# ahoynodnarb/minidiff

Measured on AMD Instinct MI355X. Metric: forward+backward passes/sec on 4096x4096 fp32 matmul+elementwise graph, higher is better.
Workload: dtype f32

## Files before the change

minidiff_amd/csrc/gemm_bf16x3.hip:

```cpp
#include "md_hip.h"
#include "md_bf16x3.h"
#include "md_bf16x3_layout.h"

namespace {

typedef __attribute__((address_space(3))) void bx_lds_void;
typedef __attribute__((address_space(1))) const void bx_gbl_void;
typedef __bf16 bx_bf16x8 __attribute__((ext_vector_type(8)));
typedef int bx_i32x4 __attribute__((ext_vector_type(4)));
typedef float bx_f32x4 __attribute__((ext_vector_type(4)));
typedef float bx_f32x16 __attribute__((ext_vector_type(16)));

constexpr int BX_BM = 256, BX_BN = 128, BX_BK = 32;
constexpr int BX_NT = 512;
constexpr int BX_ROWB = BX_BK * 2;

__device__ __forceinline__ bool bx_split8(const float (&x)[8], bx_i32x4 *q1, bx_i32x4 *q2, bx_i32x4 *q3) {
  bool bad = false;
  uint32_t h[3][8];
#pragma unroll
  for (int j = 0; j < 8; ++j) {
    uint32_t p1, p2, p3;
    bad |= md_bf16x3_split(x[j], &p1, &p2, &p3);
    h[0][j] = p1 >> 16; h[1][j] = p2 >> 16; h[2][j] = p3 >> 16;
  }
  bx_i32x4 *q[3] = {q1, q2, q3};
#pragma unroll
  for (int p = 0; p < 3; ++p)
#pragma unroll
    for (int w = 0; w < 4; ++w) (*q[p])[w] = (int)(h[p][2 * w] | (h[p][2 * w + 1] << 16));
  return bad;
}

__global__ void __launch_bounds__(256) k_bf16x3_split_rows(const float *__restrict__ src, int64_t rows, int64_t K, int64_t rs, char *__restrict__ dst,
                                                           int64_t plane, unsigned *flag) {
  bool bad = false;
  const int64_t k = ((int64_t)blockIdx.x * 256 + threadIdx.x) * 8;
  if (k < K) {
    for (int64_t r = blockIdx.y; r < rows; r += gridDim.y) {
      const bx_f32x4 lo = *(const bx_f32x4 *)(src + r * rs + k), hi = *(const bx_f32x4 *)(src + r * rs + k + 4);
      const float x[8] = {lo[0], lo[1], lo[2], lo[3], hi[0], hi[1], hi[2], hi[3]};
      bx_i32x4 q1, q2, q3;
      bad |= bx_split8(x, &q1, &q2, &q3);
      char *d = dst + md_bf16x3_plane_off(r, k, K * 2, 64);
      *(bx_i32x4 *)d = q1; *(bx_i32x4 *)(d + plane) = q2; *(bx_i32x4 *)(d + 2 * plane) = q3;
    }
  }
  if (__syncthreads_or(bad) && threadIdx.x == 0) atomicOr(flag, 1u);
}

__global__ void __launch_bounds__(256) k_bf16x3_split_rows_kt(const float *__restrict__ src, int64_t rows, int64_t K, int64_t rs, char *__restrict__ dst,
                                                              int64_t plane, unsigned *flag) {
  bool bad = false;
  const int l = threadIdx.x & 63, w = threadIdx.x >> 6;
  const int64_t k = (((int64_t)blockIdx.x * 4 + w) * 8 + (l >> 3)) * 32 + (l & 3) * 8;
  if (k < K) {
    for (int64_t r = (int64_t)blockIdx.y * 2 + ((l >> 2) & 1); r < rows; r += (int64_t)gridDim.y * 2) {
      const bx_f32x4 lo = *(const bx_f32x4 *)(src + r * rs + k), hi = *(const bx_f32x4 *)(src + r * rs + k + 4);
      const float x[8] = {lo[0], lo[1], lo[2], lo[3], hi[0], hi[1], hi[2], hi[3]};
      bx_i32x4 q1, q2, q3;
      bad |= bx_split8(x, &q1, &q2, &q3);
      char *d = dst + md_bf16x3_plane_off(r, k, 64, rows * 64);
      *(bx_i32x4 *)d = q1; *(bx_i32x4 *)(d + plane) = q2; *(bx_i32x4 *)(d + 2 * plane) = q3;
    }
  }
  if (__syncthreads_or(bad) && threadIdx.x == 0) atomicOr(flag, 1u);
}

__global__ void __launch_bounds__(256) k_bf16x3_split_cols(const float *__restrict__ src, int64_t rows, int64_t K, int64_t ks, char *__restrict__ dst,
                                                           int64_t plane, int64_t prs, int64_t pks, unsigned *flag) {
  __shared__ float T[32][66];
  const int t = threadIdx.x;
  for (int64_t kb = blockIdx.y; kb < K / 32; kb += gridDim.y) {
    const int64_t r0 = (int64_t)blockIdx.x * 64, k0 = kb * 32;
#pragma unroll
    for (int i = 0; i < 2; ++i) {
      const int idx = t + 256 * i, kk = idx >> 4, r4 = (idx & 15) * 4;
      const bx_f32x4 v = *(const bx_f32x4 *)(src + (k0 + kk) * ks + r0 + r4);
      T[kk][r4] = v[0]; T[kk][r4 + 1] = v[1]; T[kk][r4 + 2] = v[2]; T[kk][r4 + 3] = v[3];
    }
    __syncthreads();
    const int kg = t & 3, r = t >> 2;
    float x[8];
#pragma unroll
    for (int j = 0; j < 8; ++j) x[j] = T[kg * 8 + j][r];
    bx_i32x4 q1, q2, q3;
    const bool bad = bx_split8(x, &q1, &q2, &q3);
    char *d = dst + md_bf16x3_plane_off(r0 + r, k0 + kg * 8, prs, pks);
    *(bx_i32x4 *)d = q1; *(bx_i32x4 *)(d + plane) = q2; *(bx_i32x4 *)(d + 2 * plane) = q3;
    if (__syncthreads_or(bad) && t == 0) atomicOr(flag, 1u);
  }
}

template <int NP>
__device__ __forceinline__ bool bxp_split8(const float (&x)[8], bx_i32x4 (&q)[NP]) {
  bool bad = false;
  uint32_t h[NP][8];
#pragma unroll
  for (int j = 0; j < 8; ++j) {
    uint32_t p[2];
    bad |= md_bf16x3_split_rn(x[j], NP, &p[0], &p[1]);
#pragma unroll
    for (int i = 0; i < NP; ++i) h[i][j] = p[i] >> 16;
  }
#pragma unroll
  for (int p = 0; p < NP; ++p)
#pragma unroll
    for (int w = 0; w < 4; ++w) q[p][w] = (int)(h[p][2 * w] | (h[p][2 * w + 1] << 16));
  return bad;
}
template <int NP>
__device__ __forceinline__ void bxp_put(char *d, int64_t plane, const bx_i32x4 (&q)[NP]) {
#pragma unroll
  for (int p = 0; p < NP; ++p) *(bx_i32x4 *)(d + p * plane) = q[p];
}

template <int NP>
__global__ void __launch_bounds__(256) k_bf16xp_split_rows(const float *__restrict__ src, int64_t rows, int64_t K, int64_t rs, char *__restrict__ dst,
                                                           int64_t plane, unsigned *flag) {
  bool bad = false;
  const int64_t k = ((int64_t)blockIdx.x * 256 + threadIdx.x) * 8;
  if (k < K) {
    for (int64_t r = blockIdx.y; r < rows; r += gridDim.y) {
      const bx_f32x4 lo = *(const bx_f32x4 *)(src + r * rs + k), hi = *(const bx_f32x4 *)(src + r * rs + k + 4);
      const float x[8] = {lo[0], lo[1], lo[2], lo[3], hi[0], hi[1], hi[2], hi[3]};
      bx_i32x4 q[NP];
      bad |= bxp_split8<NP>(x, q);
      bxp_put<NP>(dst + md_bf16x3_plane_off(r, k, K * 2, 64), plane, q);
    }
  }
  if (__syncthreads_or(bad) && threadIdx.x == 0) atomicOr(flag, 1u);
}

template <int NP>
__global__ void __launch_bounds__(256) k_bf16xp_split_rows_kt(const float *__restrict__ src, int64_t rows, int64_t K, int64_t rs, char *__restrict__ dst,
                                                              int64_t plane, unsigned *flag) {
  bool bad = false;
  const int l = threadIdx.x & 63, w = threadIdx.x >> 6;
  const int64_t k = (((int64_t)blockIdx.x * 4 + w) * 8 + (l >> 3)) * 32 + (l & 3) * 8;
  if (k < K) {
    for (int64_t r = (int64_t)blockIdx.y * 2 + ((l >> 2) & 1); r < rows; r += (int64_t)gridDim.y * 2) {
      const bx_f32x4 lo = *(const bx_f32x4 *)(src + r * rs + k), hi = *(const bx_f32x4 *)(src + r * rs + k + 4);
      const float x[8] = {lo[0], lo[1], lo[2], lo[3], hi[0], hi[1], hi[2], hi[3]};
      bx_i32x4 q[NP];
      bad |= bxp_split8<NP>(x, q);
      bxp_put<NP>(dst + md_bf16x3_plane_off(r, k, 64, rows * 64), plane, q);
    }
  }
  if (__syncthreads_or(bad) && threadIdx.x == 0) atomicOr(flag, 1u);
}

template <int NP>
__global__ void __launch_bounds__(256) k_bf16xp_split_cols(const float *__restrict__ src, int64_t rows, int64_t K, int64_t ks, char *__restrict__ dst,
                                                           int64_t plane, int64_t prs, int64_t pks, unsigned *flag) {
  __shared__ float T[32][66];
  const int t = threadIdx.x;
  for (int64_t kb = blockIdx.y; kb < K / 32; kb += gridDim.y) {
    const int64_t r0 = (int64_t)blockIdx.x * 64, k0 = kb * 32;
#pragma unroll
    for (int i = 0; i < 2; ++i) {
      const int idx = t + 256 * i, kk = idx >> 4, r4 = (idx & 15) * 4;
      const bx_f32x4 v = *(const bx_f32x4 *)(src + (k0 + kk) * ks + r0 + r4);
      T[kk][r4] = v[0]; T[kk][r4 + 1] = v[1]; T[kk][r4 + 2] = v[2]; T[kk][r4 + 3] = v[3];
    }
    __syncthreads();
    const int kg = t & 3, r = t >> 2;
    float x[8];
#pragma unroll
    for (int j = 0; j < 8; ++j) x[j] = T[kg * 8 + j][r];
    bx_i32x4 q[NP];
    const bool bad = bxp_split8<NP>(x, q);
    bxp_put<NP>(dst + md_bf16x3_plane_off(r0 + r, k0 + kg * 8, prs, pks), plane, q);
    if (__syncthreads_or(bad) && t == 0) atomicOr(flag, 1u);
  }
}

struct Bx3Args {
  const char *A, *B;
  float *C;
  int64_t K, c_ms;
  int64_t a_plane, b_plane;
  int64_t rs, a_kstep, b_kstep;
  int tiles_m, tiles_n, gm;
  const unsigned *flag;
  unsigned long long *stamp;
};

__device__ __forceinline__ const char *bx_uniform(const char *p) {
  uint32_t lo = (uint32_t)(uintptr_t)p, hi = (uint32_t)((uintptr_t)p >> 32);
  asm("" : "+s"(lo), "+s"(hi));
  return reinterpret_cast<const char *>(((uintptr_t)hi << 32) | lo);
}

__device__ __forceinline__ void bx_piece(const char *P, int64_t rs, int64_t row, int64_t kstep, int kt, uint32_t lane_off, char *S) {
  uint32_t off = lane_off;
  asm("" : "+v"(off) : "s"(kt));
  const char *src = bx_uniform(P + row * rs + kt * kstep) + off;
  __builtin_amdgcn_global_load_lds((bx_gbl_void *)src, (bx_lds_void *)S, 16, 0, 0);
}

struct Bx3Bufs { char *a[3], *b[3]; };

template <int NP>
__device__ __forceinline__ void bx_stage(const Bx3Args &g, int64_t m0, int64_t n0, int kt, const Bx3Bufs &S, uint32_t lane_off) {
  const int wave = __builtin_amdgcn_readfirstlane(threadIdx.x >> 6);
#pragma unroll
  for (int p = 0; p < NP; ++p) {
#pragma unroll
    for (int i = 0; i < 2; ++i) bx_piece(g.A + p * g.a_plane, g.rs, m0 + 16 * (wave + 8 * i), g.a_kstep, kt, lane_off, S.a[p] + (wave + 8 * i) * 1024);
    bx_piece(g.B + p * g.b_plane, g.rs, n0 + 16 * wave, g.b_kstep, kt, lane_off, S.b[p] + wave * 1024);
  }
}

__device__ __forceinline__ bx_bf16x8 bx_frag(const char *S, int rb, int s) {
  const int l = threadIdx.x & 63, r = rb + (l & 31), c = 2 * s + (l >> 5);
  return __builtin_bit_cast(bx_bf16x8, *(const bx_i32x4 *)(S + r * BX_ROWB + ((c ^ ((r >> 2) & 3)) << 4)));
}

__device__ __forceinline__ bx_bf16x8 bx_frag_at(const char *S, uint32_t off, int half) {
  return __builtin_bit_cast(bx_bf16x8, *(const bx_i32x4 *)(S + off + half * 32 * BX_ROWB));
}
__device__ __forceinline__ uint32_t bx_read_off(int rb, int s) {
  const int l = threadIdx.x & 63, r = rb + (l & 31), c = 2 * s + (l >> 5);
  return (uint32_t)(r * BX_ROWB + ((c ^ ((r >> 2) & 3)) << 4));
}

template <int NP, int NPROD>
__device__ __forceinline__ void bx_mma(const Bx3Bufs &S, int wm, int wn, bx_f32x16 (&acc)[2][2]) {
  bx_f32x16 part[2][2];
#pragma unroll
  for (int i = 0; i < 2; ++i)
#pragma unroll
    for (int j = 0; j < 2; ++j)
#pragma unroll
      for (int e = 0; e < 16; ++e) part[i][j][e] = 0;
#pragma unroll
  for (int s = 0; s < 2; ++s) {
    bx_bf16x8 a[NP][2], b[NP][2];
#pragma unroll
    for (int p = 0; p < NP; ++p)
#pragma unroll
      for (int i = 0; i < 2; ++i) {
        a[p][i] = bx_frag(S.a[p], wm * 64 + i * 32, s);
        b[p][i] = bx_frag(S.b[p], wn * 64 + i * 32, s);
      }
    constexpr int PA[6] = {0, 0, 1, 0, 1, 2}, PB[6] = {0, 1, 0, 2, 1, 0};
#pragma unroll
    for (int q = 0; q < NPROD; ++q)
#pragma unroll
      for (int i = 0; i < 2; ++i)
#pragma unroll
        for (int j = 0; j < 2; ++j) part[i][j] = __builtin_amdgcn_mfma_f32_32x32x16_bf16(a[PA[q]][i], b[PB[q]][j], part[i][j], 0, 0, 0);
  }
#pragma unroll
  for (int i = 0; i < 2; ++i)
#pragma unroll
    for (int j = 0; j < 2; ++j) acc[i][j] += part[i][j];
}

struct Bx3Src { const char *a[3][2], *b[3]; };
struct Bx3Dst { char *a[3][2], *b[3]; };

__device__ __forceinline__ void bx_fence() { __builtin_amdgcn_sched_barrier(0); }

__device__ __forceinline__ void bx_dma(const char *&base, int64_t step, uint32_t lane_off, char *S) {
  base = bx_uniform(base + step);
  uint32_t off = lane_off;
  asm("" : "+v"(off));
  __builtin_amdgcn_global_load_lds((bx_gbl_void *)(base + off), (bx_lds_void *)S, 16, 0, 0);
}

__device__ __forceinline__ void bx_dma_n(Bx3Src &src, const Bx3Dst &dst, int n, int64_t ka, int64_t kb, uint32_t lane_off) {
  const int p = n / 3, i = n % 3;
  if (i < 2) bx_dma(src.a[p][i], ka, lane_off, dst.a[p][i]);
  else bx_dma(src.b[p], kb, lane_off, dst.b[p]);
}

__device__ __forceinline__ void bx_fold4(bx_f32x16 &acc, const bx_f32x16 &part, int e0) {
  float r0 = acc[e0] + part[e0], r1 = acc[e0 + 1] + part[e0 + 1], r2 = acc[e0 + 2] + part[e0 + 2], r3 = acc[e0 + 3] + part[e0 + 3];
  asm volatile("" : "+v"(r0), "+v"(r1), "+v"(r2), "+v"(r3));
  acc[e0] = r0; acc[e0 + 1] = r1; acc[e0 + 2] = r2; acc[e0 + 3] = r3;
}

template <bool STAGE>
__device__ __forceinline__ void bx_tile(const Bx3Bufs &S, Bx3Src &src, const Bx3Dst &dst, int64_t ka, int64_t kb, uint32_t lane_off, const uint32_t (&rd)[4],
                                        bx_f32x16 (&acc)[2][2], bx_f32x16 &carry) {
  constexpr int PA[6] = {0, 0, 1, 0, 1, 2}, PB[6] = {0, 1, 0, 2, 1, 0};
  bx_f32x16 part[2][2];
  bx_bf16x8 a0[3][2], b0[3][2], a1[3][2], b1[3][2];
  uint32_t ra0 = rd[0], ra1 = rd[1], rb0 = rd[2], rb1 = rd[3];
  asm volatile("" : "+v"(ra0), "+v"(ra1), "+v"(rb0), "+v"(rb1));
  a0[0][0] = bx_frag_at(S.a[0], ra0, 0); b0[0][0] = bx_frag_at(S.b[0], rb0, 0); b0[0][1] = bx_frag_at(S.b[0], rb0, 1); a0[0][1] = bx_frag_at(S.a[0], ra0, 1);
  b0[1][0] = bx_frag_at(S.b[1], rb0, 0); b0[1][1] = bx_frag_at(S.b[1], rb0, 1);
  a0[1][0] = bx_frag_at(S.a[1], ra0, 0); a0[1][1] = bx_frag_at(S.a[1], ra0, 1);
  b0[2][0] = bx_frag_at(S.b[2], rb0, 0); b0[2][1] = bx_frag_at(S.b[2], rb0, 1);
  a0[2][0] = bx_frag_at(S.a[2], ra0, 0); a0[2][1] = bx_frag_at(S.a[2], ra0, 1);
  bx_fence();
#pragma unroll
  for (int q = 0; q < 6; ++q)
#pragma unroll
    for (int i = 0; i < 2; ++i)
#pragma unroll
      for (int j = 0; j < 2; ++j) {
        const int n = q * 4 + i * 2 + j;
        if (q == 0) {
          const bx_f32x16 zero = {0, 0, 0, 0, 0, 0, 0, 0, 0, 0, 0, 0, 0, 0, 0, 0};
          part[i][j] = __builtin_amdgcn_mfma_f32_32x32x16_bf16(a0[0][i], b0[0][j], zero, 0, 0, 0);
        } else {
          part[i][j] = __builtin_amdgcn_mfma_f32_32x32x16_bf16(a0[PA[q]][i], b0[PB[q]][j], part[i][j], 0, 0, 0);
        }
        if (n < 4) bx_fold4(acc[1][1], carry, 4 * n);
        if (n >= 4 && n <= 12) {
          if (STAGE) bx_dma_n(src, dst, n - 4, ka, kb, lane_off);
          if (n == 12) __builtin_amdgcn_s_waitcnt(0xC07F);
        }
        switch (n) {
          case 12: a1[0][0] = bx_frag_at(S.a[0], ra1, 0); b1[0][0] = bx_frag_at(S.b[0], rb1, 0); break;
          case 13: b1[1][0] = bx_frag_at(S.b[1], rb1, 0); a1[1][0] = bx_frag_at(S.a[1], ra1, 0); break;
          case 14: b1[2][0] = bx_frag_at(S.b[2], rb1, 0); a1[2][0] = bx_frag_at(S.a[2], ra1, 0); break;
          case 15: b1[0][1] = bx_frag_at(S.b[0], rb1, 1); b1[1][1] = bx_frag_at(S.b[1], rb1, 1); break;
          case 16: b1[2][1] = bx_frag_at(S.b[2], rb1, 1); a1[0][1] = bx_frag_at(S.a[0], ra1, 1); break;
          case 17: a1[1][1] = bx_frag_at(S.a[1], ra1, 1); a1[2][1] = bx_frag_at(S.a[2], ra1, 1); break;
          default: break;
        }
        bx_fence();
      }
#pragma unroll
  for (int t = 0; t < 4; ++t) {
    const int i = t >> 1, j = t & 1;
#pragma unroll
    for (int q = 0; q < 6; ++q) {
      part[i][j] = __builtin_amdgcn_mfma_f32_32x32x16_bf16(a1[PA[q]][i], b1[PB[q]][j], part[i][j], 0, 0, 0);
      if (t > 0 && q >= 2) bx_fold4(acc[(t - 1) >> 1][(t - 1) & 1], part[(t - 1) >> 1][(t - 1) & 1], 4 * (q - 2));
      bx_fence();
    }
  }
  carry = part[1][1];
}

__device__ __forceinline__ void bx2_barrier() {
  bx_fence();
  asm volatile("" ::: "memory");
  __builtin_amdgcn_s_barrier();
  asm volatile("" ::: "memory");
  bx_fence();
}

template <bool STAGE>
__device__ __forceinline__ void bx2_tile(const Bx3Bufs &S, Bx3Src &src, const Bx3Dst &dst, int64_t ka, int64_t kb, uint32_t lane_off, const uint32_t (&rd)[4],
                                         bx_f32x16 (&acc)[2][2], bx_f32x16 (&part)[2][2]) {
  constexpr int PA[6] = {0, 0, 1, 0, 1, 2}, PB[6] = {0, 1, 0, 2, 1, 0};
  constexpr int NL = 3, CSTEP = 4;
#pragma unroll
  for (int s = 0; s < 2; ++s) {
    bx_bf16x8 a[3][2], b[3][2];
    uint32_t ra = rd[s], rb = rd[2 + s];
    asm volatile("" : "+v"(ra), "+v"(rb));
    a[0][0] = bx_frag_at(S.a[0], ra, 0); b[0][0] = bx_frag_at(S.b[0], rb, 0); b[0][1] = bx_frag_at(S.b[0], rb, 1); a[0][1] = bx_frag_at(S.a[0], ra, 1);
    b[1][0] = bx_frag_at(S.b[1], rb, 0); b[1][1] = bx_frag_at(S.b[1], rb, 1);
    a[1][0] = bx_frag_at(S.a[1], ra, 0); a[1][1] = bx_frag_at(S.a[1], ra, 1);
    b[2][0] = bx_frag_at(S.b[2], rb, 0); b[2][1] = bx_frag_at(S.b[2], rb, 1);
    a[2][0] = bx_frag_at(S.a[2], ra, 0); a[2][1] = bx_frag_at(S.a[2], ra, 1);
    bx_fence();
    if (s == 0) {
      if (STAGE) {
#pragma unroll
        for (int n = 0; n < NL; ++n) bx_dma_n(src, dst, n, ka, kb, lane_off);
      }
      bx_fence();
#pragma unroll
      for (int t = 0; t < 4; ++t)
#pragma unroll
        for (int e = 0; e < 16; e += 4) bx_fold4(acc[t >> 1][t & 1], part[t >> 1][t & 1], e);
      bx_fence();
    }
    if (s == 0) __builtin_amdgcn_s_waitcnt(0xC07F);
    else __builtin_amdgcn_s_waitcnt(0x0070);
    bx2_barrier();
#pragma unroll
    for (int q = 0; q < 6; ++q)
#pragma unroll
      for (int i = 0; i < 2; ++i)
#pragma unroll
        for (int j = 0; j < 2; ++j) {
          const int n = q * 4 + i * 2 + j;
          if (s == 0 && q == 0) {
            const bx_f32x16 zero = {0, 0, 0, 0, 0, 0, 0, 0, 0, 0, 0, 0, 0, 0, 0, 0};
            part[i][j] = __builtin_amdgcn_mfma_f32_32x32x16_bf16(a[0][i], b[0][j], zero, 0, 0, 0);
          } else {
            part[i][j] = __builtin_amdgcn_mfma_f32_32x32x16_bf16(a[PA[q]][i], b[PB[q]][j], part[i][j], 0, 0, 0);
          }
          if (STAGE && s == 0 && n % CSTEP == 1 && NL + n / CSTEP < 9) bx_dma_n(src, dst, NL + n / CSTEP, ka, kb, lane_off);
          bx_fence();
        }
    bx2_barrier();
  }
}

__device__ __forceinline__ void bx_origin(const Bx3Args &g, int64_t *m0, int64_t *n0) {
  const int nwg = g.tiles_m * g.tiles_n, bid = blockIdx.x, xcd = bid & 7, q = nwg >> 3, r = nwg & 7;
  const int wg = (xcd < r ? xcd * (q + 1) : r * (q + 1) + (xcd - r) * q) + (bid >> 3);
  int tm, tn;
  md_bf16x3_tile(wg, g.tiles_m, g.tiles_n, g.gm, &tm, &tn);
  *m0 = (int64_t)tm * BX_BM; *n0 = (int64_t)tn * BX_BN;
}
__device__ __forceinline__ void bx_write_c(const Bx3Args &g, int64_t m0, int64_t n0, int wm, int wn, int l, const bx_f32x16 (&acc)[2][2]) {
#pragma unroll
  for (int i = 0; i < 2; ++i)
#pragma unroll
    for (int j = 0; j < 2; ++j)
#pragma unroll
      for (int e = 0; e < 16; ++e) {
        const int64_t m = m0 + wm * 64 + i * 32 + (e & 3) + 8 * (e >> 2) + 4 * (l >> 5), n = n0 + wn * 64 + j * 32 + (l & 31);
        g.C[m * g.c_ms + n] = acc[i][j][e];
      }
}

template <int LOOP, bool STAMP = false>
__global__ void __launch_bounds__(BX_NT) k_gemm_bf16x3(Bx3Args g) {
  __shared__ __attribute__((aligned(16))) char sA00[BX_BM * BX_ROWB];
  __shared__ __attribute__((aligned(16))) char sA01[BX_BM * BX_ROWB];
  __shared__ __attribute__((aligned(16))) char sA02[BX_BM * BX_ROWB];
  __shared__ __attribute__((aligned(16))) char sB00[BX_BN * BX_ROWB];
  __shared__ __attribute__((aligned(16))) char sB01[BX_BN * BX_ROWB];
  __shared__ __attribute__((aligned(16))) char sB02[BX_BN * BX_ROWB];
  __shared__ __attribute__((aligned(16))) char sA10[BX_BM * BX_ROWB];
  __shared__ __attribute__((aligned(16))) char sA11[BX_BM * BX_ROWB];
  __shared__ __attribute__((aligned(16))) char sA12[BX_BM * BX_ROWB];
  __shared__ __attribute__((aligned(16))) char sB10[BX_BN * BX_ROWB];
  __shared__ __attribute__((aligned(16))) char sB11[BX_BN * BX_ROWB];
  __shared__ __attribute__((aligned(16))) char sB12[BX_BN * BX_ROWB];
  if (g.flag && *g.flag != 0) return;
  const Bx3Bufs S0{{sA00, sA01, sA02}, {sB00, sB01, sB02}}, S1{{sA10, sA11, sA12}, {sB10, sB11, sB12}};
  const int nwg = g.tiles_m * g.tiles_n, bid = blockIdx.x, xcd = bid & 7, q = nwg >> 3, r = nwg & 7;
  const int wg = (xcd < r ? xcd * (q + 1) : r * (q + 1) + (xcd - r) * q) + (bid >> 3);
  int tm, tn;
  md_bf16x3_tile(wg, g.tiles_m, g.tiles_n, g.gm, &tm, &tn);
  const int64_t m0 = (int64_t)tm * BX_BM, n0 = (int64_t)tn * BX_BN;
  const int wave = threadIdx.x >> 6, wm = wave >> 1, wn = wave & 1, l = threadIdx.x & 63;
  const int nk = (int)(g.K / BX_BK);
  const uint32_t lane_off = (uint32_t)((l >> 2) * g.rs + (((l & 3) ^ ((l >> 4) & 3)) << 4));
  bx_f32x16 acc[2][2];
#pragma unroll
  for (int i = 0; i < 2; ++i)
#pragma unroll
    for (int j = 0; j < 2; ++j)
#pragma unroll
      for (int e = 0; e < 16; ++e) acc[i][j][e] = 0;
  unsigned long long st_c = 0, st_r = 0;
  if constexpr (STAMP) {
    st_c = __builtin_amdgcn_s_memtime(); st_r = __builtin_amdgcn_s_memrealtime();
    __builtin_amdgcn_s_waitcnt(0xC07F);
  }
  if constexpr (LOOP == 0) {
    bx_stage<3>(g, m0, n0, 0, S0, lane_off);
    for (int kt = 0; kt < nk; kt += 2) {
      __syncthreads();
      if (kt + 1 < nk) bx_stage<3>(g, m0, n0, kt + 1, S1, lane_off);
      bx_mma<3, 6>(S0, wm, wn, acc);
      if (kt + 1 >= nk) break;
      __syncthreads();
      if (kt + 2 < nk) bx_stage<3>(g, m0, n0, kt + 2, S0, lane_off);
      bx_mma<3, 6>(S1, wm, wn, acc);
    }
  } else {
    const int uw = __builtin_amdgcn_readfirstlane(wave);
    const int64_t rs = g.rs, ka = g.a_kstep, kb = g.b_kstep;
    Bx3Src src;
    Bx3Dst d0, d1;
#pragma unroll
    for (int p = 0; p < 3; ++p) {
#pragma unroll
      for (int i = 0; i < 2; ++i) {
        src.a[p][i] = bx_uniform(g.A + p * g.a_plane + (m0 + 16 * (uw + 8 * i)) * rs);
        d0.a[p][i] = S0.a[p] + (uw + 8 * i) * 1024;
        d1.a[p][i] = S1.a[p] + (uw + 8 * i) * 1024;
      }
      src.b[p] = bx_uniform(g.B + p * g.b_plane + (n0 + 16 * uw) * rs);
      d0.b[p] = S0.b[p] + uw * 1024;
      d1.b[p] = S1.b[p] + uw * 1024;
    }
    const uint32_t rd[4] = {bx_read_off(wm * 64, 0), bx_read_off(wm * 64, 1), bx_read_off(wn * 64, 0), bx_read_off(wn * 64, 1)};
    if constexpr (LOOP == 1) {
      bx_f32x16 carry = {0, 0, 0, 0, 0, 0, 0, 0, 0, 0, 0, 0, 0, 0, 0, 0};
#pragma unroll
      for (int n = 0; n < 9; ++n) bx_dma_n(src, d0, n, 0, 0, lane_off);
      int kt = 0;
      for (; kt + 2 < nk; kt += 2) {
        __syncthreads();
        bx_tile<true>(S0, src, d1, ka, kb, lane_off, rd, acc, carry);
        __syncthreads();
        bx_tile<true>(S1, src, d0, ka, kb, lane_off, rd, acc, carry);
      }
      __syncthreads();
      if (kt + 1 < nk) {
        bx_tile<true>(S0, src, d1, ka, kb, lane_off, rd, acc, carry);
        __syncthreads();
        bx_tile<false>(S1, src, d0, 0, 0, lane_off, rd, acc, carry);
      } else {
        bx_tile<false>(S0, src, d1, 0, 0, lane_off, rd, acc, carry);
      }
#pragma unroll
      for (int e = 0; e < 16; e += 4) bx_fold4(acc[1][1], carry, e);
    } else {
      const int half = uw >> 2;
      bx_f32x16 part[2][2];
#pragma unroll
      for (int i = 0; i < 2; ++i)
#pragma unroll
        for (int j = 0; j < 2; ++j)
#pragma unroll
          for (int e = 0; e < 16; ++e) part[i][j][e] = 0;
#pragma unroll
      for (int n = 0; n < 9; ++n) bx_dma_n(src, d0, n, 0, 0, lane_off);
      __builtin_amdgcn_s_waitcnt(0x0070);
      bx2_barrier();
      if (half) bx2_barrier();
      int kt = 0;
      for (; kt + 2 < nk; kt += 2) {
        bx2_tile<true>(S0, src, d1, ka, kb, lane_off, rd, acc, part);
        bx2_tile<true>(S1, src, d0, ka, kb, lane_off, rd, acc, part);
      }
      if (kt + 1 < nk) {
        bx2_tile<true>(S0, src, d1, ka, kb, lane_off, rd, acc, part);
        bx2_tile<false>(S1, src, d0, 0, 0, lane_off, rd, acc, part);
      } else {
        bx2_tile<false>(S0, src, d1, 0, 0, lane_off, rd, acc, part);
      }
#pragma unroll
      for (int t = 0; t < 4; ++t)
#pragma unroll
        for (int e = 0; e < 16; e += 4) bx_fold4(acc[t >> 1][t & 1], part[t >> 1][t & 1], e);
      if (!half) bx2_barrier();
    }
  }
  if constexpr (STAMP) {
    if (threadIdx.x == 0) {
      g.stamp[2 * blockIdx.x] = __builtin_amdgcn_s_memtime() - st_c;
      g.stamp[2 * blockIdx.x + 1] = __builtin_amdgcn_s_memrealtime() - st_r;
    }
  }
#pragma unroll
  for (int i = 0; i < 2; ++i)
#pragma unroll
    for (int j = 0; j < 2; ++j)
#pragma unroll
      for (int e = 0; e < 16; ++e) {
        const int64_t m = m0 + wm * 64 + i * 32 + (e & 3) + 8 * (e >> 2) + 4 * (l >> 5), n = n0 + wn * 64 + j * 32 + (l & 31);
        g.C[m * g.c_ms + n] = acc[i][j][e];
      }
}

template <int NPROD>
__global__ void __launch_bounds__(BX_NT) k_gemm_bf16xp(Bx3Args g) {
  constexpr int NP = NPROD == 1 ? 1 : 2;
  __shared__ __attribute__((aligned(16))) char sA0[NP * BX_BM * BX_ROWB];
  __shared__ __attribute__((aligned(16))) char sB0[NP * BX_BN * BX_ROWB];
  __shared__ __attribute__((aligned(16))) char sA1[NP * BX_BM * BX_ROWB];
  __shared__ __attribute__((aligned(16))) char sB1[NP * BX_BN * BX_ROWB];
  if (g.flag && *g.flag != 0) return;
  const Bx3Bufs S0{{sA0, sA0 + (NP - 1) * BX_BM * BX_ROWB, nullptr}, {sB0, sB0 + (NP - 1) * BX_BN * BX_ROWB, nullptr}};
  const Bx3Bufs S1{{sA1, sA1 + (NP - 1) * BX_BM * BX_ROWB, nullptr}, {sB1, sB1 + (NP - 1) * BX_BN * BX_ROWB, nullptr}};
  int64_t m0, n0;
  bx_origin(g, &m0, &n0);
  const int wave = threadIdx.x >> 6, wm = wave >> 1, wn = wave & 1, l = threadIdx.x & 63;
  const int nk = (int)(g.K / BX_BK);
  const uint32_t lane_off = (uint32_t)((l >> 2) * g.rs + (((l & 3) ^ ((l >> 4) & 3)) << 4));
  bx_f32x16 acc[2][2];
#pragma unroll
  for (int i = 0; i < 2; ++i)
#pragma unroll
    for (int j = 0; j < 2; ++j)
#pragma unroll
      for (int e = 0; e < 16; ++e) acc[i][j][e] = 0;
  bx_stage<NP>(g, m0, n0, 0, S0, lane_off);
  for (int kt = 0; kt < nk; kt += 2) {
    __syncthreads();
    if (kt + 1 < nk) bx_stage<NP>(g, m0, n0, kt + 1, S1, lane_off);
    bx_mma<NP, NPROD>(S0, wm, wn, acc);
    if (kt + 1 >= nk) break;
    __syncthreads();
    if (kt + 2 < nk) bx_stage<NP>(g, m0, n0, kt + 2, S0, lane_off);
    bx_mma<NP, NPROD>(S1, wm, wn, acc);
  }
  bx_write_c(g, m0, n0, wm, wn, l, acc);
}

}

int md_gemm_bf16x3_split(const float *src, bool k_contig, int64_t rows, int64_t K, int64_t stride, void *planes, unsigned *flag, int layout, int nplanes) {
  const int64_t plane = rows * K * 2;
  char *dst = (char *)planes;
  if (k_contig && layout) {
    const dim3 grid((unsigned)((K / 32 + 31) / 32), (unsigned)(rows / 2 < 65535 ? rows / 2 : 65535));
    switch (nplanes) {
      case 1: k_bf16xp_split_rows_kt<1><<<grid, 256, 0, md_stream()>>>(src, rows, K, stride, dst, plane, flag); break;
      case 2: k_bf16xp_split_rows_kt<2><<<grid, 256, 0, md_stream()>>>(src, rows, K, stride, dst, plane, flag); break;
      default: k_bf16x3_split_rows_kt<<<grid, 256, 0, md_stream()>>>(src, rows, K, stride, dst, plane, flag); break;
    }
  } else if (k_contig) {
    const dim3 grid((unsigned)((K / 8 + 255) / 256), (unsigned)(rows < 65535 ? rows : 65535));
    switch (nplanes) {
      case 1: k_bf16xp_split_rows<1><<<grid, 256, 0, md_stream()>>>(src, rows, K, stride, dst, plane, flag); break;
      case 2: k_bf16xp_split_rows<2><<<grid, 256, 0, md_stream()>>>(src, rows, K, stride, dst, plane, flag); break;
      default: k_bf16x3_split_rows<<<grid, 256, 0, md_stream()>>>(src, rows, K, stride, dst, plane, flag); break;
    }
  } else {
    const dim3 grid((unsigned)(rows / 64), (unsigned)(K / 32 < 65535 ? K / 32 : 65535));
    const int64_t prs = md_bf16x3_row_stride(layout, K), pks = md_bf16x3_k_step(layout, rows);
    switch (nplanes) {
      case 1: k_bf16xp_split_cols<1><<<grid, 256, 0, md_stream()>>>(src, rows, K, stride, dst, plane, prs, pks, flag); break;
      case 2: k_bf16xp_split_cols<2><<<grid, 256, 0, md_stream()>>>(src, rows, K, stride, dst, plane, prs, pks, flag); break;
      default: k_bf16x3_split_cols<<<grid, 256, 0, md_stream()>>>(src, rows, K, stride, dst, plane, prs, pks, flag); break;
    }
  }
  return MD_LAUNCH_CHECK("matmul(bf16x3 split)");
}

int md_gemm_bf16x3(const void *a_planes, const void *b_planes, float *c, int64_t M, int64_t N, int64_t K, int64_t c_ms, const unsigned *flag, int loop,
                   int layout, int band, int products, unsigned long long *stamp) {
  Bx3Args a{};
  a.A = (const char *)a_planes; a.B = (const char *)b_planes; a.C = c;
  a.K = K; a.c_ms = c_ms;
  a.a_plane = M * K * 2; a.b_plane = N * K * 2;
  a.rs = md_bf16x3_row_stride(layout, K); a.a_kstep = md_bf16x3_k_step(layout, M); a.b_kstep = md_bf16x3_k_step(layout, N);
  a.tiles_m = (int)(M / BX_BM); a.tiles_n = (int)(N / BX_BN);
  a.gm = md_bf16x3_band(a.tiles_m, MD_NUM_CUS / 8, band);
  a.flag = flag;
  a.stamp = stamp;
  md_opt_table()[MD_OPT_GEMM_BF16X3_RUNS] += 1;
  const dim3 grid((unsigned)(a.tiles_m * a.tiles_n));
  if (products == 1) MD_LAUNCH(k_gemm_bf16xp<1>, grid, BX_NT, a);
  else if (products == 3) MD_LAUNCH(k_gemm_bf16xp<3>, grid, BX_NT, a);
  else if (stamp && loop == 0) MD_LAUNCH((k_gemm_bf16x3<0, true>), grid, BX_NT, a);
  else if (stamp && loop == 2) MD_LAUNCH((k_gemm_bf16x3<2, true>), grid, BX_NT, a);
  else if (stamp) MD_LAUNCH((k_gemm_bf16x3<1, true>), grid, BX_NT, a);
  else if (loop == 0) MD_LAUNCH(k_gemm_bf16x3<0>, grid, BX_NT, a);
  else if (loop == 2) MD_LAUNCH(k_gemm_bf16x3<2>, grid, BX_NT, a);
  else MD_LAUNCH(k_gemm_bf16x3<1>, grid, BX_NT, a);
  return MD_LAUNCH_CHECK("matmul(f32 as bf16x3)");
}
```

minidiff_amd/csrc/md_options.h:

```cpp
#pragma once
#include <stdint.h>
#include <stdlib.h>
#include <string.h>

#define MD_OPTION_LIST(X)                                                                                                        \
                                                                                    \
  X(PINNED_CAP, "pinned_cap", (int64_t)4 << 30, 'c')                  \
  X(JIT, "jit", 1, 'c')                                      \
  X(JIT_VERBOSE, "jit_verbose", 0, 'c')                                           \
  X(INDEX_DEFER, "index_defer", 0, 'c')                 \
                                                              \
  X(JIT_MIN, "jit_min", 1 << 18, 'x')                                   \
  X(COMM_PRIORITY, "comm_priority", 0, 'x')                         \
  X(MAX_BLOCKS, "max_blocks", 0, 'x')                                      \
  X(NT, "nt", -1, 'x')                                      \
  X(GEMM_CFG, "gemm_cfg", -1, 'x')                                  \
  X(GEMM_GLDS, "gemm_glds", 1, 'x')                                                   \
  X(GEMM_NBUF, "gemm_nbuf", 0, 'x')                     \
  X(GEMM_PEEL, "gemm_peel", 1, 'x')                            \
  X(GEMM_TT_SWAP, "gemm_tt_swap", 1, 'x')                                \
  X(GEMM_REPACK, "gemm_repack", 1, 'x')                         \
  X(GEMM_SUPER, "gemm_super", 8, 'x')                                      \
  X(GEMM_SPLITK, "gemm_splitk", 1, 'x')                                                                                         \
  X(GEMM_STAMP, "gemm_stamp", 0, 'x')                                                  \
  X(GEMM_F64_MFMA, "gemm_f64_mfma", 1, 'x')                                                                                     \
  X(GEMM_SKINNY, "gemm_skinny", 1, 'x')                                \
  X(GEMM_WIDEN, "gemm_widen", 1, 'x')                   \
  X(GEMM_NARROW_SKINNY, "gemm_narrow_skinny", 1, 'x')   \
  X(GEMM_NARROW_THIN_RUNS, "gemm_narrow_thin_runs", 0, 'x')  \
  X(GEMM_BF16X3, "gemm_bf16x3", 1, 'x')                 \
  X(GEMM_BF16X3_RUNS, "gemm_bf16x3_runs", 0, 'x')       \
  X(GEMM_BF16X3_LOOP, "gemm_bf16x3_loop", 2, 'x')       \
  X(GEMM_BF16X3_BAND, "gemm_bf16x3_band", 0, 'x')       \
  X(GEMM_BF16X3_PLANES, "gemm_bf16x3_planes", 1, 'x')   \
  X(GEMM_PRODUCTS, "gemm_products", 6, 'x')             \
  X(JIT_U, "jit_u", 0, 'x')                             \
  X(JIT_BLOCKS, "jit_blocks", 0, 'x')                                       \
  X(JIT_AXES_WIDE, "jit_axes_wide", 0, 'x')             \
  X(SWEEP_NB, "sweep_nb", 0, 'x')                                         \
  X(SWEEP_RU, "sweep_ru", 0, 'x')                                                                                               \
  X(SWEEP_NT_STORE, "sweep_nt_store", 1, 'x')                                                                                   \
  X(ROWS_WAVE, "rows_wave", 1, 'x')                                                                                             \
  X(COLS_NB, "cols_nb", 0, 'x')                                                                                                 \
  X(ROWS_BLOCKS, "rows_blocks", 0, 'x')                                          \
  X(ARG_BLOCKS, "arg_blocks", 0, 'x')                                   \
  X(ARG_BATCHED, "arg_batched", 1, 'x')                 \
  X(VAR_BATCHED, "var_batched", 1, 'x')                      \
  X(GATHER_RUNS, "gather_runs", 1, 'x')                                                                                         \
  X(SCATTER_CENSUS, "scatter_census", 1, 'x')                                                                                   \
  X(SCATTER_SORTED, "scatter_sorted", 1, 'x')

enum MdOptId {
#define MD_OPT_ENUM(ID, name, dflt, kind) MD_OPT_##ID,
  MD_OPTION_LIST(MD_OPT_ENUM)
#undef MD_OPT_ENUM
  MD_OPT_COUNT
};

struct MdOptDef {
  const char *name;
  int64_t dflt;
  char kind;
};

inline const MdOptDef *md_opt_defs() {
  static const MdOptDef defs[MD_OPT_COUNT] = {
#define MD_OPT_DEF(ID, name, dflt, kind) {name, (int64_t)(dflt), kind},
      MD_OPTION_LIST(MD_OPT_DEF)
#undef MD_OPT_DEF
  };
  return defs;
}

inline int64_t *md_opt_table() {
  static int64_t table[MD_OPT_COUNT];
  static const bool loaded = [] {
    const MdOptDef *d = md_opt_defs();
    const char *ex = getenv("MDHIP_EXPERIMENTS");
    const bool experiments = ex && ex[0] == '1' && ex[1] == 0;
    for (int i = 0; i < MD_OPT_COUNT; ++i) {
      table[i] = d[i].dflt;
      if (d[i].kind == 'x' && !experiments) continue;
      char env[64] = "MDHIP_";
      size_t n = strlen(env);
      for (const char *p = d[i].name; *p && n + 1 < sizeof env; ++p) env[n++] = (char)((*p >= 'a' && *p <= 'z') ? *p - 32 : *p);
      env[n] = 0;
      if (const char *v = getenv(env)) table[i] = (int64_t)atoll(v);
    }
    return true;
  }();
  (void)loaded;
  return table;
}
inline int64_t md_opt(int id) { return md_opt_table()[id]; }
inline int md_opt_find(const char *name) {
  const MdOptDef *d = md_opt_defs();
  for (int i = 0; i < MD_OPT_COUNT; ++i)
    if (strcmp(d[i].name, name) == 0) return i;
  return -1;
}
```

Before: 608.7.

## Add 16x16x32 MFMA bf16x3 loop variant with split accumulators and make default

```diff
diff --git a/minidiff_amd/csrc/gemm_bf16x3.hip b/minidiff_amd/csrc/gemm_bf16x3.hip
--- a/minidiff_amd/csrc/gemm_bf16x3.hip
+++ b/minidiff_amd/csrc/gemm_bf16x3.hip
@@ -397,6 +397,86 @@
   }
 }
 
+__device__ __forceinline__ uint32_t bx3_swz(int g) { return (0x78u >> (2 * g)) & 3u; }
+
+__device__ __forceinline__ uint32_t bx3_read_off(int rb) {
+  const int l = threadIdx.x & 63, r = rb + (l & 15), c = l >> 4;
+  return (uint32_t)(r * BX_ROWB + ((c ^ bx3_swz((r >> 2) & 3)) << 4));
+}
+__device__ __forceinline__ bx_bf16x8 bx3_frag_at(const char *S, uint32_t off, int i) {
+  return __builtin_bit_cast(bx_bf16x8, *(const bx_i32x4 *)(S + off + i * 16 * BX_ROWB));
+}
+
+__device__ __forceinline__ void bx3_fold4(bx_f32x4 &acc, const bx_f32x4 &part) {
+  float r0 = acc[0] + part[0], r1 = acc[1] + part[1], r2 = acc[2] + part[2], r3 = acc[3] + part[3];
+  asm volatile("" : "+v"(r0), "+v"(r1), "+v"(r2), "+v"(r3));
+  acc[0] = r0; acc[1] = r1; acc[2] = r2; acc[3] = r3;
+}
+
+template <bool STAGE>
+__device__ __forceinline__ void bx3_tile(const Bx3Bufs &S, Bx3Src &src, const Bx3Dst &dst, int64_t ka, int64_t kb, uint32_t lane_off, const uint32_t (&rd)[2],
+                                         bx_f32x4 (&acc)[4][4], bx_f32x4 (&part)[2][4]) {
+  constexpr int PA[6] = {0, 0, 1, 0, 1, 2}, PB[6] = {0, 1, 0, 2, 1, 0};
+  constexpr int NL = 3, CSTEP = 8;
+  bx_bf16x8 b[3][4];
+#pragma unroll
+  for (int h = 0; h < 2; ++h) {
+    bx_bf16x8 a[3][2];
+    uint32_t ra = rd[0], rb = rd[1];
+    asm volatile("" : "+v"(ra), "+v"(rb));
+    if (h == 0) {
+#pragma unroll
+      for (int i = 0; i < 2; ++i) a[0][i] = bx3_frag_at(S.a[0], ra, i);
+#pragma unroll
+      for (int j = 0; j < 4; ++j) b[0][j] = bx3_frag_at(S.b[0], rb, j);
+#pragma unroll
+      for (int j = 0; j < 4; ++j) b[1][j] = bx3_frag_at(S.b[1], rb, j);
+#pragma unroll
+      for (int i = 0; i < 2; ++i) a[1][i] = bx3_frag_at(S.a[1], ra, i);
+#pragma unroll
+      for (int j = 0; j < 4; ++j) b[2][j] = bx3_frag_at(S.b[2], rb, j);
+#pragma unroll
+      for (int i = 0; i < 2; ++i) a[2][i] = bx3_frag_at(S.a[2], ra, i);
+    } else {
+#pragma unroll
+      for (int p = 0; p < 3; ++p)
+#pragma unroll
+        for (int i = 0; i < 2; ++i) a[p][i] = bx3_frag_at(S.a[p], ra, 2 + i);
+    }
+    bx_fence();
+    if (h == 0 && STAGE) {
+#pragma unroll
+      for (int n = 0; n < NL; ++n) bx_dma_n(src, dst, n, ka, kb, lane_off);
+    }
+    bx_fence();
+#pragma unroll
+    for (int i = 0; i < 2; ++i)
+#pragma unroll
+      for (int j = 0; j < 4; ++j) bx3_fold4(acc[2 * (1 - h) + i][j], part[i][j]);
+    bx_fence();
+    if (h == 0) __builtin_amdgcn_s_waitcnt(0xC07F);
+    else __builtin_amdgcn_s_waitcnt(0x0070);
+    bx2_barrier();
+#pragma unroll
+    for (int q = 0; q < 6; ++q)
+#pragma unroll
+      for (int i = 0; i < 2; ++i)
+#pragma unroll
+        for (int j = 0; j < 4; ++j) {
+          const int n = q * 8 + i * 4 + j;
+          if (q == 0) {
+            const bx_f32x4 zero = {0, 0, 0, 0};
+            part[i][j] = __builtin_amdgcn_mfma_f32_16x16x32_bf16(a[0][i], b[0][j], zero, 0, 0, 0);
+          } else {
+            part[i][j] = __builtin_amdgcn_mfma_f32_16x16x32_bf16(a[PA[q]][i], b[PB[q]][j], part[i][j], 0, 0, 0);
+          }
+          if (STAGE && h == 0 && n % CSTEP == 1 && NL + n / CSTEP < 9) bx_dma_n(src, dst, NL + n / CSTEP, ka, kb, lane_off);
+          bx_fence();
+        }
+    bx2_barrier();
+  }
+}
+
 __device__ __forceinline__ void bx_origin(const Bx3Args &g, int64_t *m0, int64_t *n0) {
   const int nwg = g.tiles_m * g.tiles_n, bid = blockIdx.x, xcd = bid & 7, q = nwg >> 3, r = nwg & 7;
   const int wg = (xcd < r ? xcd * (q + 1) : r * (q + 1) + (xcd - r) * q) + (bid >> 3);
@@ -412,6 +492,82 @@
 #pragma unroll
       for (int e = 0; e < 16; ++e) {
         const int64_t m = m0 + wm * 64 + i * 32 + (e & 3) + 8 * (e >> 2) + 4 * (l >> 5), n = n0 + wn * 64 + j * 32 + (l & 31);
+        g.C[m * g.c_ms + n] = acc[i][j][e];
+      }
+}
+
+template <bool STAMP>
+__device__ __forceinline__ void bx3_run(const Bx3Args &g, const Bx3Bufs &S0, const Bx3Bufs &S1, int64_t m0, int64_t n0) {
+  const int wave = threadIdx.x >> 6, wm = wave >> 1, wn = wave & 1, l = threadIdx.x & 63;
+  const int nk = (int)(g.K / BX_BK);
+  const uint32_t lane_off = (uint32_t)((l >> 2) * g.rs + (((l & 3) ^ bx3_swz((l >> 4) & 3)) << 4));
+  bx_f32x4 acc[4][4], part[2][4];
+#pragma unroll
+  for (int i = 0; i < 4; ++i)
+#pragma unroll
+    for (int j = 0; j < 4; ++j)
+#pragma unroll
+      for (int e = 0; e < 4; ++e) {
+        acc[i][j][e] = 0;
+        if (i < 2) part[i][j][e] = 0;
+      }
+  unsigned long long st_c = 0, st_r = 0;
+  if constexpr (STAMP) {
+    st_c = __builtin_amdgcn_s_memtime(); st_r = __builtin_amdgcn_s_memrealtime();
+    __builtin_amdgcn_s_waitcnt(0xC07F);
+  }
+  const int uw = __builtin_amdgcn_readfirstlane(wave);
+  const int64_t rs = g.rs, ka = g.a_kstep, kb = g.b_kstep;
+  Bx3Src src;
+  Bx3Dst d0, d1;
+#pragma unroll
+  for (int p = 0; p < 3; ++p) {
+#pragma unroll
+    for (int i = 0; i < 2; ++i) {
+      src.a[p][i] = bx_uniform(g.A + p * g.a_plane + (m0 + 16 * (uw + 8 * i)) * rs);
+      d0.a[p][i] = S0.a[p] + (uw + 8 * i) * 1024;
+      d1.a[p][i] = S1.a[p] + (uw + 8 * i) * 1024;
+    }
+    src.b[p] = bx_uniform(g.B + p * g.b_plane + (n0 + 16 * uw) * rs);
+    d0.b[p] = S0.b[p] + uw * 1024;
+    d1.b[p] = S1.b[p] + uw * 1024;
+  }
+  const uint32_t rd[2] = {bx3_read_off(wm * 64), bx3_read_off(wn * 64)};
+  const int half = uw >> 2;
+#pragma unroll
+  for (int n = 0; n < 9; ++n) bx_dma_n(src, d0, n, 0, 0, lane_off);
+  __builtin_amdgcn_s_waitcnt(0x0070);
+  bx2_barrier();
+  if (half) bx2_barrier();
+  int kt = 0;
+  for (; kt + 2 < nk; kt += 2) {
+    bx3_tile<true>(S0, src, d1, ka, kb, lane_off, rd, acc, part);
+    bx3_tile<true>(S1, src, d0, ka, kb, lane_off, rd, acc, part);
+  }
+  if (kt + 1 < nk) {
+    bx3_tile<true>(S0, src, d1, ka, kb, lane_off, rd, acc, part);
+    bx3_tile<false>(S1, src, d0, 0, 0, lane_off, rd, acc, part);
+  } else {
+    bx3_tile<false>(S0, src, d1, 0, 0, lane_off, rd, acc, part);
+  }
+#pragma unroll
+  for (int i = 0; i < 2; ++i)
+#pragma unroll
+    for (int j = 0; j < 4; ++j) bx3_fold4(acc[2 + i][j], part[i][j]);
+  if (!half) bx2_barrier();
+  if constexpr (STAMP) {
+    if (threadIdx.x == 0) {
+      g.stamp[2 * blockIdx.x] = __builtin_amdgcn_s_memtime() - st_c;
+      g.stamp[2 * blockIdx.x + 1] = __builtin_amdgcn_s_memrealtime() - st_r;
+    }
+  }
+#pragma unroll
+  for (int i = 0; i < 4; ++i)
+#pragma unroll
+    for (int e = 0; e < 4; ++e)
+#pragma unroll
+      for (int j = 0; j < 4; ++j) {
+        const int64_t m = m0 + wm * 64 + i * 16 + 4 * (l >> 4) + e, n = n0 + wn * 64 + j * 16 + (l & 15);
         g.C[m * g.c_ms + n] = acc[i][j][e];
       }
 }
@@ -437,6 +593,10 @@
   int tm, tn;
   md_bf16x3_tile(wg, g.tiles_m, g.tiles_n, g.gm, &tm, &tn);
   const int64_t m0 = (int64_t)tm * BX_BM, n0 = (int64_t)tn * BX_BN;
+  if constexpr (LOOP == 3) {
+    bx3_run<STAMP>(g, S0, S1, m0, n0);
+    return;
+  }
   const int wave = threadIdx.x >> 6, wm = wave >> 1, wn = wave & 1, l = threadIdx.x & 63;
   const int nk = (int)(g.K / BX_BK);
   const uint32_t lane_off = (uint32_t)((l >> 2) * g.rs + (((l & 3) ^ ((l >> 4) & 3)) << 4));
@@ -634,9 +794,11 @@
   else if (products == 3) MD_LAUNCH(k_gemm_bf16xp<3>, grid, BX_NT, a);
   else if (stamp && loop == 0) MD_LAUNCH((k_gemm_bf16x3<0, true>), grid, BX_NT, a);
   else if (stamp && loop == 2) MD_LAUNCH((k_gemm_bf16x3<2, true>), grid, BX_NT, a);
+  else if (stamp && loop == 3) MD_LAUNCH((k_gemm_bf16x3<3, true>), grid, BX_NT, a);
   else if (stamp) MD_LAUNCH((k_gemm_bf16x3<1, true>), grid, BX_NT, a);
   else if (loop == 0) MD_LAUNCH(k_gemm_bf16x3<0>, grid, BX_NT, a);
   else if (loop == 2) MD_LAUNCH(k_gemm_bf16x3<2>, grid, BX_NT, a);
+  else if (loop == 3) MD_LAUNCH(k_gemm_bf16x3<3>, grid, BX_NT, a);
   else MD_LAUNCH(k_gemm_bf16x3<1>, grid, BX_NT, a);
   return MD_LAUNCH_CHECK("matmul(f32 as bf16x3)");
 }
diff --git a/minidiff_amd/csrc/md_options.h b/minidiff_amd/csrc/md_options.h
--- a/minidiff_amd/csrc/md_options.h
+++ b/minidiff_amd/csrc/md_options.h
@@ -30,7 +30,7 @@
   X(GEMM_NARROW_THIN_RUNS, "gemm_narrow_thin_runs", 0, 'x')  \
   X(GEMM_BF16X3, "gemm_bf16x3", 1, 'x')                 \
   X(GEMM_BF16X3_RUNS, "gemm_bf16x3_runs", 0, 'x')       \
-  X(GEMM_BF16X3_LOOP, "gemm_bf16x3_loop", 2, 'x')       \
+  X(GEMM_BF16X3_LOOP, "gemm_bf16x3_loop", 3, 'x')       \
   X(GEMM_BF16X3_BAND, "gemm_bf16x3_band", 0, 'x')       \
   X(GEMM_BF16X3_PLANES, "gemm_bf16x3_planes", 1, 'x')   \
   X(GEMM_PRODUCTS, "gemm_products", 6, 'x')             \
```

After: 649.8, median of 6. +6.8%, better.
